# succinctlabs/kzg-rs

Measured on AMD Instinct MI355X. Metric: blobs/sec verify_blob_kzg_proof_batch, higher is better.
Workload: dtype u32 limbs (255-bit Fr / 381-bit Fp modular integers); 1 GPU; verify_blob_kzg_proof_batch, batches of 1024 synthetic blobs (4096 Fr each), device-resident, known-tau test setup (BASELINE.json configs[1]); one step = one launch group of 256 independent batches = 262144 blobs per GPU; blobs_per_gpu_per_batch=1024, batch=1024, parallelism=shard-by-blob x1, groups_in_flight=4

## Files before the change

kzg_rs_amd/csrc/capi_verify.hpp:

```cpp

static KzgRet launch_evaluate(const KzgSettings* s, const void* d_blobs, const Fr* d_z, Fr* d_y, uint32_t* d_status, size_t T, bool alone = false,
                              bool stamp = false) {
    unsigned long long* const kt = stamp && s->ws.d_ktime.p ? s->ws.d_ktime.p + 4 : nullptr;
    HIPCHK(s->d_eval_scratch.grow(eval_scratch_words(std::max<size_t>(T, 1024))));
    const unsigned per_lane = (unsigned)((T + 63) / 64);
    hipLaunchKernelGGL(k_eval_powers, dim3(per_lane), dim3(64), 0, s->s1, d_z, s->d_eval_scratch.p, (int)T);
    const unsigned eval_blocks = (unsigned)((T + EVAL_BLOBS_PER_BLOCK - 1) / EVAL_BLOBS_PER_BLOCK);
    static const long pad_opt = ab_int("eval_lds_pad", -1);
    const size_t lds_pad = pad_opt >= 0 ? (size_t)std::min(120L * 1024, pad_opt) : alone ? 0 : 16384;
    size_t spread_lds = eval_blocks <= (unsigned)s->n_cus ? (size_t)EVAL_SPREAD_LDS : lds_pad;
    if (spread_lds && DYN_LDS(k_blob_evaluate_t<true>, spread_lds) != hipSuccess) {
        (void)hipGetLastError();
        spread_lds = 0;
    }
    hipLaunchKernelGGL(k_blob_evaluate_t<true>, dim3(eval_blocks), dim3(64 * EVAL_BLOBS_PER_BLOCK), spread_lds, s->s1,
                       (const uint8_t*)d_blobs, EvalTables{s->t->d_eval_a.p, s->t->d_eval_b.p, s->t->d_eval_c.p}, s->d_eval_scratch.p, d_status, (int)T, kt);
    hipLaunchKernelGGL(k_eval_finish, dim3(per_lane), dim3(64), 0, s->s1, s->d_eval_scratch.p, s->t->d_M29.p, d_y, (int)T);
    return KZG_OK;
}

static KzgRet launch_challenge(const KzgSettings* s, const void* d_blobs, const void* d_commitments, Fr* d_z, size_t T, hipStream_t st = nullptr) {
    if (!st) st = s->s1;
    static const int forced = opt_is("challenge_kernel", "lane") ? 1 : opt_is("challenge_kernel", "split") ? 2 : opt_is("challenge_kernel", "split2") ? 3 : 0;
    const uint8_t *bl = (const uint8_t*)d_blobs, *cm = (const uint8_t*)d_commitments;
    const int form = forced ? forced : T <= 16384 ? 3 : T <= 49152 ? 2 : 1;
    s->ws.ktime_valid = false;
    if (form == 1) {
        unsigned long long* kt = s->ws.d_ktime.p;
        if (kt) {
            HIPCHK(hipMemsetAsync(kt, 0, 32, st));
            s->ws.ktime_valid = true;
        }
        hipLaunchKernelGGL(k_blob_challenge_t<4>, dim3((unsigned)((T + 255) / 256)), dim3(256), 0, st, bl, cm, d_z, (int)T, kt);
    } else if (form == 2) {
        hipLaunchKernelGGL(k_blob_challenge_split, dim3((unsigned)((T + 63) / 64)), dim3(128), 0, st, bl, cm, d_z, (int)T);
    } else {
        hipLaunchKernelGGL(k_blob_challenge_split2_t<false>, dim3((unsigned)((T + 63) / 64)), dim3(192), 0, st, bl, cm, d_z, (int)T, 0, 1024, (uint32_t*)nullptr);
    }
    HIPCHK(hipGetLastError());
    return KZG_OK;
}

enum { STAGE_NONE = 0, STAGE_BLOBS = 1, STAGE_CP = 2 };
static KzgRet ws_reserve(const KzgSettings* s, size_t T, size_t B, int stage) {
    Workspace& w = s->ws;
    if (T > w.cap_n || B > w.cap_b) {
        size_t capT = T > w.cap_n ? T : w.cap_n, capB = B > w.cap_b ? B : w.cap_b;
        w.reset();
        if (capT < 16) capT = 16;
        const size_t np = 2 * capT + 1;
        const size_t nsc = 2 * capT + capB;
        const size_t nterm = 4 * capT + 2 * capB;
        HIPCHK(w.d_z.alloc(capT));
        HIPCHK(w.d_y.alloc(capT));
        HIPCHK(w.d_scalars.alloc(nsc));
        HIPCHK(w.d_partial.alloc((capT + 255) / 256 + capB));
        HIPCHK(w.d_r.alloc(capB));
        HIPCHK(w.d_status.alloc(capT));
        HIPCHK(w.d_pflag.alloc(np));
        HIPCHK(w.d_term_point.alloc(nterm));
        HIPCHK(w.d_term_scalar.alloc(nterm));
        HIPCHK(w.d_sorted.alloc(MSM_WINDOWS * nterm));
        HIPCHK(w.d_points.alloc(np));
        HIPCHK(w.d_window.alloc(2 * MSM_WINDOWS * capB));
        HIPCHK(w.d_window_sl.alloc(2 * MSM_WINDOWS * MSM_MAX_SLICES * 4));
        HIPCHK(w.d_mult.alloc(MULT_ENTRY_BYTES * std::max((size_t)MSM_CHUNKS * np, (size_t)MSM_CHUNKS_LATENCY * std::min(np, (size_t)(2 * LATENCY_MAX_BLOBS + 1)))));
        HIPCHK(w.d_ab.alloc(2 * capB));
        HIPCHK(w.d_ktime.alloc(16));
        if (msm_affine_enabled()) HIPCHK(w.d_jtmp.alloc(np));
        HIPCHK(w.d_parts.alloc(2 * capB * MAX_WORLD));
        HIPCHK(w.d_send.alloc(2 * MAX_WORLD));
        HIPCHK(w.d_slp_in.alloc(6 * capB));
        HIPCHK(w.d_slp_out.alloc(6 * capB));
        HIPCHK(w.d_bytes.alloc(96 * np));
        HIPCHK(w.d_records.alloc(160 * capT));
        HIPCHK(w.d_sha_mid.alloc(8 * std::min(capT, (size_t)SLICED_MAX_BLOBS)));
        w.off_r = 256 * capT + 4096;
        w.off_part = w.off_r + 32 * capB;
        w.off_out = w.off_part + 288 * capB;
        w.off_parts = w.off_out + 288 * capB;
        HIPCHK(w.h_buf.alloc(w.off_parts + 288 * capB * MAX_WORLD));
        w.cap_n = capT;
        w.cap_b = capB;
    }
    const size_t n_stage = std::max<size_t>(T, 4);
    if (stage != STAGE_NONE) HIPCHK(w.d_stage_cp.grow(96 * n_stage));
    if (stage == STAGE_BLOBS) HIPCHK(w.d_stage_blobs.grow((size_t)BLOB_BYTES * n_stage));
    return KZG_OK;
}

static int msm_chunks_per_block(size_t B) {
    static const int forced = [] {
        const int v = (int)ab_int("msm_cpb", 0);
        return (v == 1 || v == 2 || v == 4) ? v : 0;
    }();
    if (forced) return forced;
    return B >= 32 ? 4 : B >= 16 ? 2 : 1;
}

static KzgRet msm_save_grow(const KzgSettings* s, size_t bytes) {
    HIPCHK(s->ws.d_msm_save.grow((bytes + 3) / 4));
    return KZG_OK;
}
static size_t msm_save_bytes(const Workspace& w) { return w.d_msm_save.cap * 4; }
static KzgRet msm_save_reserve(const KzgSettings* s, unsigned gx, unsigned gy, unsigned gz) {
    const size_t layer = msm_save_layer_bytes(gx, gy, MSM_SAVE2_WORDS);
    return msm_save_grow(s, std::max(layer, std::min(layer * gz, (size_t)512 << 20)));
}

static KzgRet run_msm(const KzgSettings* s, size_t n, size_t B) {
    Workspace& w = s->ws;
    const int T = (int)(n * B), mt = (int)(2 * n + 1);
    hipLaunchKernelGGL(k_batch_terms, dim3((unsigned)((n + 255) / 256), (unsigned)B), dim3(256), 0, s->s1, w.d_term_point.p,
                       w.d_term_scalar.p, (int)n, T, mt);
    MsmDesc d{};
    d.mult = w.d_mult.p;
    d.pflag = w.d_pflag.p;
    d.scalars = w.d_scalars.p;
    d.term_point = w.d_term_point.p;
    d.term_scalar = w.d_term_scalar.p;
    d.sorted = w.d_sorted.p;
    d.window_sums = w.d_window.p;
    d.nterms[0] = (int)n;
    d.nterms[1] = (int)(2 * n + 1);
    d.max_terms = mt;
    d.stride = 2 * T + 1;
    d.ktime = w.kstamps_valid ? w.d_ktime.p + 8 : nullptr;
    d.chunks = w.chunks;
    d.chunks_per_block = w.chunks == MSM_CHUNKS ? msm_chunks_per_block(B) : 1;
    static const int msm_flags = ab_flag("msm_xcd", true) ? MSM_FLAG_XCD : 0;
    d.flags = msm_flags;
    const unsigned slots = d.chunks / d.chunks_per_block, W = MSM_WINDOWS / d.chunks;
    unsigned S = 1;
    while (S < MSM_MAX_SLICES && W * slots * 2 * B * S < 768 && n / (2 * S) >= 1024 && 2 * S * B <= 128) S *= 2;
    static const unsigned latency_slices = [] {
        const unsigned v = (unsigned)ab_int("msm_latency_slices", 0);
        return v == 1 || v == 2 || v == 4 || v == 8 ? v : 4u;
    }();
    if (d.chunks != MSM_CHUNKS && S == 1 && n >= 256 && B <= 4) S = latency_slices;
    const size_t lds_cap = msm_lds_sort_capacity<Curve29>();
    auto slice_terms = [&](unsigned S_) { return ((size_t)mt + S_ - 1) / S_ * (size_t)d.chunks_per_block; };
    while (S < MSM_MAX_SLICES && slice_terms(S) > lds_cap && n / (2 * S) >= 1024 && 2 * S * B <= 128) S *= 2;
    const bool lds_sort = slice_terms(S) + 1 <= lds_cap;
    d.slices = (int)S;
    d.window_sums = S > 1 ? w.d_window_sl.p : w.d_window.p;
    HIPCHK(hipEventRecord(s->ev[2], s->s1));
    const int nsc = (int)(B * (2 * n + 1));
    hipLaunchKernelGGL(k_glv_split, dim3((unsigned)((nsc + 255) / 256)), dim3(256), 0, s->s1, w.d_scalars.p, nsc);
    const unsigned gz = (unsigned)(2 * B * S);
    KzgRet rc_save = msm_save_reserve(s, W, slots, gz);
    if (rc_save != KZG_OK) return rc_save;
    if (w.mult_affine) {
        if (lds_sort) msm_window_launch<Curve29Aff, true>(d, W, slots, gz, w.d_msm_save.p, msm_save_bytes(w), s->s1);
        else msm_window_launch<Curve29Aff, false>(d, W, slots, gz, w.d_msm_save.p, msm_save_bytes(w), s->s1);
    } else {
        static const bool tree_quads = ab_flag("msm_tree_quads", true);
        if (tree_quads && d.chunks != MSM_CHUNKS && B <= 4) {
            if (lds_sort) msm_window_launch<Curve29Quads, true>(d, W, slots, gz, w.d_msm_save.p, msm_save_bytes(w), s->s1);
            else msm_window_launch<Curve29Quads, false>(d, W, slots, gz, w.d_msm_save.p, msm_save_bytes(w), s->s1);
        } else if (lds_sort) msm_window_launch<Curve29, true>(d, W, slots, gz, w.d_msm_save.p, msm_save_bytes(w), s->s1);
        else msm_window_launch<Curve29, false>(d, W, slots, gz, w.d_msm_save.p, msm_save_bytes(w), s->s1);
    }
    static const bool sum_quads = ab_flag("msm_sum_quads", true);
    if (sum_quads && W == 1 && slots * S >= 2 && slots * S <= (unsigned)SUMQ_MAX_POINTS && 2 * B < 64) {
        HIPCHK(DYN_LDS(k_msm_sum_quads, SUMQ_LDS_BYTES));
        hipLaunchKernelGGL(k_msm_sum_quads, dim3((unsigned)(2 * B)), dim3(256), SUMQ_LDS_BYTES, s->s1, d.window_sums, w.d_ab.p, (int)(slots * S));
        HIPCHK(hipGetLastError());
        HIPCHK(hipEventRecord(s->ev[3], s->s1));
        return KZG_OK;
    }
    if (S > 1)
        hipLaunchKernelGGL(k_msm_fold_slices, dim3((unsigned)(2 * B * slots * W)), dim3(64), 0, s->s1, w.d_window_sl.p, w.d_window.p, (int)S, (int)W);
    if (2 * B >= 64)
        hipLaunchKernelGGL(k_msm_combine_lanes, dim3((unsigned)((2 * B + 63) / 64)), dim3(64), 0, s->s1, w.d_window.p, w.d_ab.p, (int)slots, (int)W, (int)(2 * B));
    else
        hipLaunchKernelGGL(k_msm_combine, dim3((unsigned)(2 * B)), dim3(64), 0, s->s1, w.d_window.p, w.d_ab.p, (int)slots, (int)W);
    HIPCHK(hipGetLastError());
    HIPCHK(hipEventRecord(s->ev[3], s->s1));
    return KZG_OK;
}

static KzgRet launch_decode(const KzgSettings* s, const void* d_commitments, const void* d_proofs, size_t T, bool behind_sha = true) {
    Workspace& w = s->ws;
    const int np = (int)(2 * T + 1);
    unsigned blocks = (unsigned)((2 * T + 63) / 64);
    static const bool no_latency_layout = !ab_flag("msm_latency_layout", true);
    w.chunks = (T <= LATENCY_MAX_BLOBS && !no_latency_layout) ? MSM_CHUNKS_LATENCY : MSM_CHUNKS;
    const uint8_t *c = (const uint8_t*)d_commitments, *p = (const uint8_t*)d_proofs;
    const int n2 = (int)(2 * T);
    const size_t gen_off = w.chunks == MSM_CHUNKS ? 0 : MSM_CHUNKS;
    w.mult_affine = msm_affine_enabled() && w.chunks == MSM_CHUNKS;
    if (w.mult_affine) {
        G1Aff29Mem* mult = (G1Aff29Mem*)w.d_mult.p;
        hipLaunchKernelGGL((k_g1_decode_multiples29<MSM_CHUNKS, true>), dim3((unsigned)((2 * T + 255) / 256)), dim3(256), 256 * PARK_UINT4_PER_THREAD * sizeof(uint4), s->s2, c, p, (int)T, w.d_points.p, w.d_pflag.p, w.d_mult.p, w.d_jtmp.p, n2, np,
                           w.kstamps_valid ? w.d_ktime.p + 6 : nullptr);
        const unsigned conv_blocks = (unsigned)((n2 + 64 * AFFINE_BATCH - 1) / (64 * AFFINE_BATCH));
        hipLaunchKernelGGL(k_mult_to_affine29, dim3(conv_blocks), dim3(64), 0, s->s2, w.d_jtmp.p, w.d_pflag.p, mult, n2, np);
        HIPCHK(hipEventRecord(s->ev[10], s->s2));
        hipLaunchKernelGGL(k_set_generator_multiples<G1Aff29Mem>, dim3(1), dim3(64), 0, s->s2, w.d_points.p, w.d_pflag.p, mult,
                           (const G1Aff29Mem*)s->t->d_gen_mult_aff.p, n2, np, w.chunks);
    } else {
        G1Jac29Mem* mult = (G1Jac29Mem*)w.d_mult.p;
        hipLaunchKernelGGL(k_set_generator_multiples<G1Jac29Mem>, dim3(1), dim3(64), 0, s->s2, w.d_points.p, w.d_pflag.p, mult,
                           (const G1Jac29Mem*)s->t->d_gen_mult.p + gen_off, n2, np, w.chunks);
        static const bool dec_quads = ab_flag("decode_quads", true);
        if (dec_quads && w.chunks != MSM_CHUNKS && !behind_sha && (2 * T + DECQ_POINTS_PER_BLOCK - 1) / DECQ_POINTS_PER_BLOCK <= (size_t)s->n_cus) {
            blocks = (unsigned)((2 * T + DECQ_POINTS_PER_BLOCK - 1) / DECQ_POINTS_PER_BLOCK);
            HIPCHK(DYN_LDS(k_g1_decode_multiples29_quads<MSM_CHUNKS_LATENCY>, DECQ_LDS_BYTES));
            hipLaunchKernelGGL(k_g1_decode_multiples29_quads<MSM_CHUNKS_LATENCY>, dim3(blocks), dim3(64), DECQ_LDS_BYTES, s->s2, c, p, (int)T, w.d_points.p, w.d_pflag.p, mult, n2, np);
        } else if (w.chunks == MSM_CHUNKS_LATENCY)
            hipLaunchKernelGGL((k_g1_decode_multiples29<MSM_CHUNKS_LATENCY, false>), dim3(blocks), dim3(64), 64 * PARK_UINT4_PER_THREAD * sizeof(uint4), s->s2, c, p, (int)T, w.d_points.p, w.d_pflag.p, w.d_mult.p, (G1Jac29Mem*)nullptr, n2, np);
        else
            hipLaunchKernelGGL((k_g1_decode_multiples29<MSM_CHUNKS, false>), dim3(blocks), dim3(64), 64 * PARK_UINT4_PER_THREAD * sizeof(uint4), s->s2, c, p, (int)T, w.d_points.p, w.d_pflag.p, w.d_mult.p, (G1Jac29Mem*)nullptr, n2, np);
        HIPCHK(hipEventRecord(s->ev[10], s->s2));
    }
    HIPCHK(hipGetLastError());
    return KZG_OK;
}


static void select_streams(const KzgSettings* s, size_t T) {
    if (!s->s_plain[1]) return;
    const bool small = T <= LATENCY_MAX_BLOBS;
    if (small && !s->s_half_tried) {
        s->s_half_tried = true;
        hipDeviceProp_t prop;
        if (ab_flag("cu_mask", true) && hipGetDeviceProperties(&prop, s->device) == hipSuccess && prop.multiProcessorCount >= 64) {
            const int ncu = prop.multiProcessorCount, words = (ncu + 31) / 32;
            std::vector<uint32_t> lo(words, 0), hi(words, 0);
            for (int i = 0; i < ncu; i++) ((i < ncu / 2) ? lo : hi)[i / 32] |= 1u << (i % 32);
            if (hipExtStreamCreateWithCUMask(&s->s_half[0], words, lo.data()) != hipSuccess ||
                hipExtStreamCreateWithCUMask(&s->s_half[1], words, hi.data()) != hipSuccess) {
                (void)hipGetLastError();
                if (s->s_half[0]) (void)hipStreamDestroy(s->s_half[0]);
                s->s_half[0] = s->s_half[1] = nullptr;
            }
        }
    }
    const bool use_half = small && s->s_half[0];
    s->s1 = s->s_plain[0];
    s->s_sha = use_half ? s->s_half[0] : s->s_plain[0];
    s->s2 = use_half ? s->s_half[1] : s->s_plain[1];
}
struct ScopedS2 {
    const KzgSettings* const s;
    const hipStream_t keep;
    ScopedS2(const KzgSettings* s_, hipStream_t st) : s(s_), keep(s_->s2) { s->s2 = st; }
    ScopedS2(const ScopedS2&) = delete;
    ~ScopedS2() { s->s2 = keep; }
};

struct HostBatch {
    const uint8_t *blobs, *commitments, *proofs;
    const uint8_t* z_le = nullptr;
    hostpool::Job* z_job = nullptr;
};
static size_t host_challenge_max_blobs() {
    static const size_t v = (size_t)std::max(0L, std::min(4096L, opt_int("host_challenge_max_blobs", 256)));
    return v;
}
static unsigned host_slices(size_t n) {
    static const unsigned forced = [] {
        const unsigned v = (unsigned)opt_int("host_slices", 0);
        return v == 1 || v == 2 || v == 4 || v == 8 || v == 16 ? v : 0u;
    }();
    static const bool lane_forced = opt_str("challenge_kernel") && !opt_is("challenge_kernel", "split2");
    if (n > SLICED_MAX_BLOBS || lane_forced) return 1;
    if (forced) return forced;
    return n >= 512 ? 8 : n >= 128 ? 4 : 1;
}

static KzgRet sliced_points_copy(const KzgSettings* s, const HostBatch& host, void* d_commitments, void* d_proofs, size_t T, hipEvent_t after) {
    if (!s->s_copy) {
        HIPCHK(hipStreamCreateWithFlags(&s->s_copy, hipStreamNonBlocking));
        for (auto& e : s->ev_copy) HIPCHK(hipEventCreateWithFlags(&e, hipEventDisableTiming));
    }
    if (!s->ev_slice[0])
        for (auto& e : s->ev_slice) HIPCHK(hipEventCreate(&e));
    HIPCHK(hipStreamWaitEvent(s->s_copy, after, 0));
    HIPCHK(hipMemcpyAsync(d_commitments, host.commitments, 48 * T, hipMemcpyHostToDevice, s->s_copy));
    if (d_proofs) HIPCHK(hipMemcpyAsync(d_proofs, host.proofs, 48 * T, hipMemcpyHostToDevice, s->s_copy));
    HIPCHK(hipEventRecord(s->ev_slice[0], s->s_copy));
    return KZG_OK;
}
static KzgRet sliced_segments(const KzgSettings* s, const HostBatch& host, void* d_blobs, const void* d_commitments, Fr* d_z, size_t T, unsigned S,
                              hipStream_t st) {
    s->ws.ktime_valid = false;
    HIPCHK(hipStreamWaitEvent(st, s->ev_slice[0], 0));
    const size_t W = (size_t)BLOB_BYTES / S;
    for (unsigned j = 0; j < S; j++) {
        HIPCHK(hipMemcpy2DAsync((uint8_t*)d_blobs + j * W, BLOB_BYTES, host.blobs + j * W, BLOB_BYTES, W, T, hipMemcpyHostToDevice, s->s_copy));
        HIPCHK(hipEventRecord(s->ev_slice[1 + j], s->s_copy));
        HIPCHK(hipStreamWaitEvent(st, s->ev_slice[1 + j], 0));
        hipLaunchKernelGGL(k_blob_challenge_split2_t<true>, dim3((unsigned)((T + 63) / 64)), dim3(192), 0, st, (const uint8_t*)d_blobs,
                           (const uint8_t*)d_commitments, d_z, (int)T, (int)(1024 / S * j), (int)(1024 / S * (j + 1)), s->ws.d_sha_mid.p);
    }
    HIPCHK(hipGetLastError());
    return KZG_OK;
}

static KzgRet phase1_launch_locked(const void* d_blobs, const void* d_commitments, const void* d_proofs, size_t n, size_t B,
                                   const KzgSettings* s, const HostBatch* host = nullptr) {
    if (B > MAX_BATCHES_PER_LAUNCH) return fail(KZG_BADARGS, "more than 16384 batches in one launch group");
    Workspace& w = s->ws;
    const size_t T = n * B;
    KzgRet rc;
    select_streams(s, T);
    const unsigned S = host && !host->z_le ? host_slices(T) : 1;
    w.kstamps_valid = w.d_ktime.p != nullptr;
    if (w.kstamps_valid) HIPCHK(hipMemsetAsync(w.d_ktime.p, 0, 128, s->s1));
    HIPCHK(hipEventRecord(s->ev[0], s->s1));
    if (host && S == 1) {
        HIPCHK(hipMemcpyAsync(const_cast<void*>(d_commitments), host->commitments, 48 * T, hipMemcpyHostToDevice, s->s1));
        HIPCHK(hipMemcpyAsync(const_cast<void*>(d_proofs), host->proofs, 48 * T, hipMemcpyHostToDevice, s->s1));
        HIPCHK(hipMemcpyAsync(const_cast<void*>(d_blobs), host->blobs, (size_t)BLOB_BYTES * T, hipMemcpyHostToDevice, s->s1));
        HIPCHK(hipEventRecord(s->ev[0], s->s1));
    }
    if (host && S > 1) {
        if ((rc = sliced_points_copy(s, *host, const_cast<void*>(d_commitments), const_cast<void*>(d_proofs), T, s->ev[0])) != KZG_OK) return rc;
        HIPCHK(hipStreamWaitEvent(s->s2, s->ev_slice[0], 0));
// ... 877 lines not shown
```

kzg_rs_amd/csrc/fr29_eval_fold.hpp:

```cpp
#pragma once
#include "fr29.hpp"

namespace kzg {

template <class LoadPsum>
FR29_FN Fr29 eval_sum_psums(LoadPsum psum) {
    uint64_t acc[9];
#pragma unroll
    for (int i = 0; i < 9; i++) acc[i] = 0;
    for (int k = 0; k < 64; k++) {
        const Fr29 p = psum(k);
#pragma unroll
        for (int i = 0; i < 9; i++) fr29_acc_add(acc[i], p.l[i]);
    }
    Fr29 s;
    uint64_t c = 0;
#pragma unroll
    for (int i = 0; i < 9; i++) {
        c += acc[i];
        s.l[i] = (uint32_t)c & FR29_MASK;
        c >>= 29;
    }
    const uint32_t hi = (uint32_t)c;
    c = 0;
#pragma unroll
    for (int i = 0; i < 9; i++) {
        c += s.l[i] + (uint64_t)hi * c29::FR29_ONE[i];
        s.l[i] = i < 8 ? (uint32_t)c & FR29_MASK : (uint32_t)c;
        c >>= 29;
    }
    return s;
}

template <class LoadNode, class LoadZ, class LoadRoot, class Stack>
FR29_FN Fr29 eval_fold_nodes(LoadNode node, LoadZ zpow, LoadRoot root, Stack& st) {
    Fr29 n;
    for (int k = 0; k < 64; k++) {
        n = node(k);
        int l = 0;
        for (; (k >> l) & 1; l++) {
            const Fr29 na = st.get(l);
            n = fr29_mul2(fr29_add(na, n), zpow(6 + l), fr29_sub_biased4(na, n), root((k >> l) & ~1));
        }
        if (k != 63) st.put(l, n);
    }
    return n;
}

FR29_FN Fr29 eval_tail(const Fr29& n0, const Fr29& s, const Fr29& zr, const Fr29& z4096) {
    const Fr29 sm = fr29_mul(s, fr29_const(c29::FR29_R2));
    const Fr29 x = fr29_mul(sm, z4096);
    const Fr29 nw = fr29_sub_biased(fr29_add(fr29_mul(n0, zr), sm), x);
    return fr29_mul(nw, fr29_const(c29::FR29_INV4096_PLAIN));
}

}
```

kzg_rs_amd/csrc/fr_kernels.hpp:

```cpp
#pragma once
#include "field.hpp"
#include "fr29.hpp"
#include "fr29_eval_fold.hpp"
#include "sha256.hpp"

namespace kzg {

constexpr int FE_PER_BLOB = 4096;
constexpr int BLOB_BYTES = 131072;

__device__ __forceinline__ uint32_t bitrev12(uint32_t i) { return __brev(i) >> 20; }

__global__ void k_roots_tables(Fr* __restrict__ M, Fr* __restrict__ DM) {
    int j = blockIdx.x * blockDim.x + threadIdx.x;
    if (j >= FE_PER_BLOB) return;
    uint32_t e = bitrev12(j);
    Fr w, acc = FrF::one();
#pragma unroll
    for (int i = 0; i < 8; i++) w.l[i] = consts::FR_OMEGA_MONT[i];
    for (int b = 11; b >= 0; b--) {
        acc = FrF::sqr(acc);
        if ((e >> b) & 1) acc = FrF::mul(acc, w);
    }
    M[j] = acc;
// ... 73 lines not shown
        bswap4(w, c0); bswap4(w + 4, c1); bswap4(w + 8, L[0]); bswap4(w + 12, L[1]);
        sha256_compress(st, w);
        bswap4(w, L[2]);
        w[4] = 0x80000000u;
#pragma unroll
        for (int k = 5; k < 15; k++) w[k] = 0;
        w[15] = 131152u * 8u;
        sha256_compress(st, w);
    }
    Fr d;
#pragma unroll
    for (int k = 0; k < 8; k++) d.l[k] = st.h[7 - k];
    z_out[i] = FrF::from_mont(FrF::to_mont(d));
    if (stamp) {
        const unsigned long long clk1 = __builtin_amdgcn_s_memtime(), ref1 = __builtin_amdgcn_s_memrealtime();
        atomicMax(&ktime[1], ref1);
        atomicAdd(&ktime[2], clk1 - clk0);
        atomicAdd(&ktime[3], ref1 - ref0);
    }
}

constexpr int CHALLENGE_TILE_U4 = 2 * 16 * 64;
__global__ __launch_bounds__(128) void k_blob_challenge_split(const uint8_t* __restrict__ blobs, const uint8_t* __restrict__ commitments,
                                                              Fr* __restrict__ z_out, int n) {
    __shared__ uint4 tile[CHALLENGE_TILE_U4];
    const int lane = threadIdx.x & 63;
    const int role = __builtin_amdgcn_readfirstlane(threadIdx.x >> 6);
    int i = blockIdx.x * 64 + lane;
    const bool live = i < n;
    if (!live) i = n - 1;
    constexpr int NBLK = 2050;

    if (role == 1) {
        const uint4* blob = reinterpret_cast<const uint4*>(blobs + (size_t)i * BLOB_BYTES);
        const uint4* cm = reinterpret_cast<const uint4*>(commitments + (size_t)i * 48);
        auto emit = [=](uint32_t (&w)[16], int b) {
            uint32_t kw[64];
            sha256_schedule_kw(kw, w);
            uint4* dst = tile + (b & 1) * (16 * 64) + lane;
#pragma unroll
            for (int t = 0; t < 16; t++) dst[t * 64] = make_uint4(kw[4 * t], kw[4 * t + 1], kw[4 * t + 2], kw[4 * t + 3]);
            __syncthreads();
        };
        uint4 L[8], c0, c1;
#pragma unroll
        for (int j = 0; j < 8; j++) L[j] = blob[j];
#pragma unroll 1
        for (int m = 0; m < 1024; m++) {
            uint32_t w[16];
            if (m == 0) {
                w[0] = 0x4653424c; w[1] = 0x4f425645; w[2] = 0x52494659; w[3] = 0x5f56315f;
                w[4] = 0; w[5] = 0; w[6] = 0; w[7] = FE_PER_BLOB;
            } else {
                bswap4(w, c0);
                bswap4(w + 4, c1);
            }
            bswap4(w + 8, L[0]);
            bswap4(w + 12, L[1]);
            emit(w, 2 * m);
            bswap4(w, L[2]); bswap4(w + 4, L[3]); bswap4(w + 8, L[4]); bswap4(w + 12, L[5]);
            c0 = L[6];
            c1 = L[7];
            if (m + 1 < 1024) {
                const uint4* p = blob + 8 * (m + 1);
#pragma unroll
                for (int j = 0; j < 8; j++) L[j] = p[j];
            } else {
                L[0] = cm[0]; L[1] = cm[1]; L[2] = cm[2];
            }
            emit(w, 2 * m + 1);
        }
        {
            uint32_t w[16];
            bswap4(w, c0); bswap4(w + 4, c1); bswap4(w + 8, L[0]); bswap4(w + 12, L[1]);
            emit(w, 2048);
            bswap4(w, L[2]);
            w[4] = 0x80000000u;
#pragma unroll
            for (int k = 5; k < 15; k++) w[k] = 0;
            w[15] = 131152u * 8u;
            emit(w, 2049);
        }
        __syncthreads();
    } else {
        Sha256State st;
        sha256_init(st);
        __syncthreads();
#pragma unroll 1
        for (int b = 0; b < NBLK; b++) {
            uint32_t a = st.h[0], bb = st.h[1], c = st.h[2], d = st.h[3], e = st.h[4], f = st.h[5], g = st.h[6], h = st.h[7];
            const uint4* src = tile + (b & 1) * (16 * 64) + lane;
            uint4 kw[16];
#pragma unroll
            for (int t = 0; t < 16; t++) kw[t] = src[t * 64];
#pragma unroll
            for (int t = 0; t < 16; t++) {
                asm volatile("" : "+v"(kw[t].x), "+v"(kw[t].y), "+v"(kw[t].z), "+v"(kw[t].w));
                sha256_rounds4(a, bb, c, d, e, f, g, h, kw[t]);
            }
            st.h[0] += a; st.h[1] += bb; st.h[2] += c; st.h[3] += d; st.h[4] += e; st.h[5] += f; st.h[6] += g; st.h[7] += h;
            __syncthreads();
        }
        if (live) {
            Fr dgst;
#pragma unroll
            for (int k = 0; k < 8; k++) dgst.l[k] = st.h[7 - k];
            z_out[i] = FrF::from_mont(FrF::to_mont(dgst));
        }
    }
}

template <bool SEG>
__global__ __launch_bounds__(192) void k_blob_challenge_split2_t(const uint8_t* __restrict__ blobs, const uint8_t* __restrict__ commitments,
                                                                 Fr* __restrict__ z_out, int n, int m0_arg, int m1_arg, uint32_t* __restrict__ mid) {
    __shared__ uint4 tile[CHALLENGE_TILE_U4];
    const int lane = threadIdx.x & 63;
    const int wave = __builtin_amdgcn_readfirstlane(threadIdx.x >> 6);
    const int M0 = SEG ? m0_arg : 0, M1 = SEG ? m1_arg : 1024;
    const bool last_seg = !SEG || M1 == 1024;
    const int NBLK = 2 * (M1 - M0) + (last_seg ? 2 : 0);
    if (wave == 2) {
        int i = blockIdx.x * 64 + lane;
        if (i >= n) i = n - 1;
        const uint4* blob = reinterpret_cast<const uint4*>(blobs + (size_t)i * BLOB_BYTES);
        const uint4* cm = reinterpret_cast<const uint4*>(commitments + (size_t)i * 48);
        auto emit = [=](uint32_t (&w)[16], int b) {
            uint32_t kw[64];
            sha256_schedule_kw(kw, w);
            uint4* dst = tile + (b & 1) * (16 * 64) + lane;
#pragma unroll
            for (int t = 0; t < 16; t++) dst[t * 64] = make_uint4(kw[4 * t], kw[4 * t + 1], kw[4 * t + 2], kw[4 * t + 3]);
            __syncthreads();
        };
        uint4 L[8], c0, c1;
#pragma unroll
        for (int j = 0; j < 8; j++) L[j] = blob[8 * M0 + j];
        if (SEG && M0 > 0) {
            c0 = blob[8 * M0 - 2];
            c1 = blob[8 * M0 - 1];
        }
#pragma unroll 1
        for (int m = M0; m < M1; m++) {
            uint32_t w[16];
            if (m == 0) {
                w[0] = 0x4653424c; w[1] = 0x4f425645; w[2] = 0x52494659; w[3] = 0x5f56315f;
                w[4] = 0; w[5] = 0; w[6] = 0; w[7] = FE_PER_BLOB;
            } else {
                bswap4(w, c0);
                bswap4(w + 4, c1);
            }
            bswap4(w + 8, L[0]);
            bswap4(w + 12, L[1]);
            emit(w, 2 * (m - M0));
            bswap4(w, L[2]); bswap4(w + 4, L[3]); bswap4(w + 8, L[4]); bswap4(w + 12, L[5]);
            c0 = L[6];
            c1 = L[7];
            if (m + 1 < M1) {
                const uint4* p = blob + 8 * (m + 1);
#pragma unroll
                for (int j = 0; j < 8; j++) L[j] = p[j];
            } else if (last_seg) {
                L[0] = cm[0]; L[1] = cm[1]; L[2] = cm[2];
            }
            emit(w, 2 * (m - M0) + 1);
        }
        if (last_seg) {
            uint32_t w[16];
            bswap4(w, c0); bswap4(w + 4, c1); bswap4(w + 8, L[0]); bswap4(w + 12, L[1]);
            emit(w, 2 * (M1 - M0));
            bswap4(w, L[2]);
            w[4] = 0x80000000u;
#pragma unroll
            for (int k = 5; k < 15; k++) w[k] = 0;
            w[15] = 131152u * 8u;
            emit(w, 2 * (M1 - M0) + 1);
        }
        __syncthreads();
    } else {
        const int blob_in_block = 32 * wave + 4 * (lane >> 3) + (lane & 3);
        int i = blockIdx.x * 64 + blob_in_block;
        const bool live = i < n;
        const bool a_lane = (lane & 4) == 0;
        Sha2LaneConsts c;
        c.n1 = a_lane ? 2u : 6u;
        c.n2 = a_lane ? 13u : 11u;
        c.n3 = a_lane ? 22u : 25u;
        c.m = a_lane ? 0xffffffffu : 0u;
        uint32_t H0 = a_lane ? 0x6a09e667u : 0x510e527fu, H1 = a_lane ? 0xbb67ae85u : 0x9b05688cu, H2 = a_lane ? 0x3c6ef372u : 0x1f83d9abu,
                 H3 = a_lane ? 0xa54ff53au : 0x5be0cd19u;
        uint32_t* my_mid = SEG ? mid + 8 * (size_t)(live ? i : n - 1) + (a_lane ? 0 : 4) : nullptr;
        if (SEG && M0 > 0) {
            const uint4 q = *reinterpret_cast<const uint4*>(my_mid);
            H0 = q.x; H1 = q.y; H2 = q.z; H3 = q.w;
        }
        __syncthreads();
#pragma unroll 1
        for (int b = 0; b < NBLK; b++) {
            const uint4* src = tile + (b & 1) * (16 * 64) + blob_in_block;
            constexpr int stride = 64;
            uint32_t kw[65];
#pragma unroll
            for (int t = 0; t < 16; t++) {
                const uint4 q = src[t * stride];
                kw[4 * t] = q.x; kw[4 * t + 1] = q.y; kw[4 * t + 2] = q.z; kw[4 * t + 3] = q.w;
            }
            kw[64] = 0;
            Sha2LaneRing r;
            r.x0 = H0; r.x1 = H1; r.x2 = H2; r.dd = H3;
            r.hk = a_lane ? 0u : H3 + kw[0];
            asm volatile("" : "=v"(r.nx));
#pragma unroll
            for (int t = 0; t < 6; t++) sha256_rounds10_2lane(r, kw + 10 * t + 1, c);
            sha256_rounds4_2lane(r, kw + 61, c);
            H0 += r.x0;
            H1 += r.x1;
            H2 += r.x2;
            H3 += a_lane ? r.dd : r.hk;
            __syncthreads();
        }
        if (SEG && !last_seg) {
            if (live) *reinterpret_cast<uint4*>(my_mid) = make_uint4(H0, H1, H2, H3);
            return;
        }
        const uint32_t e0 = (uint32_t)__builtin_amdgcn_update_dpp(0, (int)H0, 0x104, 0xF, 0xF, true), e1 = (uint32_t)__builtin_amdgcn_update_dpp(0, (int)H1, 0x104, 0xF, 0xF, true);
        const uint32_t e2 = (uint32_t)__builtin_amdgcn_update_dpp(0, (int)H2, 0x104, 0xF, 0xF, true), e3 = (uint32_t)__builtin_amdgcn_update_dpp(0, (int)H3, 0x104, 0xF, 0xF, true);
        if (live && a_lane) {
            const uint32_t hh[8] = {H0, H1, H2, H3, e0, e1, e2, e3};
            Fr dgst;
#pragma unroll
            for (int k = 0; k < 8; k++) dgst.l[k] = hh[7 - k];
            z_out[i] = FrF::from_mont(FrF::to_mont(dgst));
        }
    }
}

__device__ __forceinline__ Fr fr_shfl_xor(const Fr& a, int mask) {
    Fr r;
#pragma unroll
    for (int i = 0; i < 8; i++) r.l[i] = __shfl_xor((int)a.l[i], mask, 64);
    return r;
}

struct alignas(16) Fr29Mem {
    uint32_t l[12];
};
__device__ __forceinline__ Fr29 fr29_load(const Fr29Mem* p) {
    const uint4 a = *reinterpret_cast<const uint4*>(p->l), b = *reinterpret_cast<const uint4*>(p->l + 4);
    Fr29 r;
    r.l[0] = a.x; r.l[1] = a.y; r.l[2] = a.z; r.l[3] = a.w;
    r.l[4] = b.x; r.l[5] = b.y; r.l[6] = b.z; r.l[7] = b.w;
    r.l[8] = p->l[8];
    return r;
}
__global__ void k_roots_tables29(const Fr* __restrict__ M, Fr29Mem* __restrict__ M29, Fr29Mem* __restrict__ DM29) {
    int j = blockIdx.x * blockDim.x + threadIdx.x;
    if (j >= FE_PER_BLOB) return;
    Fr w = FrF::from_mont(M[j]);
    const Fr29 r2 = fr29_const(c29::FR29_R2);
    Fr29 m = fr29_mul(fr29_from_words(w.l), r2), dm = fr29_mul(m, r2);
#pragma unroll
    for (int i = 0; i < 12; i++) {
        M29[j].l[i] = i < 9 ? m.l[i] : 0u;
        DM29[j].l[i] = i < 9 ? dm.l[i] : 0u;
    }
}

constexpr int EVAL_SLOTS = 63;
struct EvalTables {
    const uint4 *a, *b;
    const uint32_t* c;
};
__global__ void k_eval_tables(const Fr29Mem* __restrict__ M29, const Fr29Mem* __restrict__ DM29, uint4* __restrict__ ta,
                              uint4* __restrict__ tb, uint32_t* __restrict__ tc) {
    const int slot = blockIdx.x, lane = threadIdx.x;
    const Fr29Mem* e;
    if (slot < 32) {
        e = DM29 + 2 * (32 * lane + slot);
    } else {
        int L = 1, rel = slot - 32;
        while (rel >= (32 >> L)) { rel -= 32 >> L; L++; }
        const int q = (rel << L) | ((1 << L) - 1);
        e = M29 + (((32 * lane + q) >> (L - 1)) & ~1);
    }
    ta[slot * 64 + lane] = make_uint4(e->l[0], e->l[1], e->l[2], e->l[3]);
    tb[slot * 64 + lane] = make_uint4(e->l[4], e->l[5], e->l[6], e->l[7]);
    tc[slot * 64 + lane] = e->l[8];
}

struct EvalRsrc {
    __amdgpu_buffer_rsrc_t a, b, c;
};
__device__ __forceinline__ Fr29 eval_table_load(const EvalRsrc& t, int slot, uint32_t lane16, uint32_t lane4) {
    typedef uint32_t u32x4 __attribute__((ext_vector_type(4)));
    const u32x4 a = __builtin_amdgcn_raw_buffer_load_b128(t.a, lane16, slot * 1024, 0);
    const u32x4 b = __builtin_amdgcn_raw_buffer_load_b128(t.b, lane16, slot * 1024, 0);
    Fr29 r;
    r.l[0] = a.x; r.l[1] = a.y; r.l[2] = a.z; r.l[3] = a.w;
    r.l[4] = b.x; r.l[5] = b.y; r.l[6] = b.z; r.l[7] = b.w;
    r.l[8] = __builtin_amdgcn_raw_buffer_load_b32(t.c, lane4, slot * 256, 0);
    return r;
}

constexpr int EVAL_SCRATCH_WORDS = 14 * 9;
constexpr int EVAL_NODE_WORDS = 2 * 64 * 12;
__host__ __device__ inline size_t eval_nodes_offset(size_t T) { return (T * EVAL_SCRATCH_WORDS + 3) & ~(size_t)3; }
__host__ __device__ inline size_t eval_scratch_words(size_t T) { return eval_nodes_offset(T) + T * EVAL_NODE_WORDS; }
__global__ __launch_bounds__(64) void k_eval_powers(const Fr* __restrict__ z_in, uint32_t* __restrict__ scratch, int T) {
    const int b = blockIdx.x * 64 + threadIdx.x;
    if (b >= T) return;
    const Fr zin = z_in[b];
    const Fr29 r2 = fr29_const(c29::FR29_R2);
    Fr29* Z = reinterpret_cast<Fr29*>(scratch + (size_t)b * EVAL_SCRATCH_WORDS);
    Fr29 z = fr29_mul(fr29_from_words(zin.l), r2);
    Z[0] = z;
    Z[13] = fr29_mul(z, r2);
    for (int l = 1; l <= 12; l++) {
        z = fr29_mul(z, z);
        Z[l] = z;
    }
}
__global__ __launch_bounds__(64) void k_eval_finish(const uint32_t* __restrict__ scratch, const Fr29Mem* __restrict__ M29, Fr* __restrict__ y_out, int T) {
    __shared__ uint32_t zs[6][9][64], stack[6][9][64];
    const int lane = threadIdx.x, b = blockIdx.x * 64 + lane;
    if (b >= T) return;
    const uint32_t* Z = scratch + (size_t)b * EVAL_SCRATCH_WORDS;
    const Fr29Mem* nodes = reinterpret_cast<const Fr29Mem*>(scratch + eval_nodes_offset(T)) + (size_t)b * 128;
    for (int L = 6; L < 12; L++)
#pragma unroll
        for (int i = 0; i < 9; i++) zs[L - 6][i][lane] = Z[L * 9 + i];
    struct Stack {
        uint32_t (*s)[9][64];
        int lane;
        __device__ Fr29 get(int l) const {
            Fr29 r;
#pragma unroll
            for (int i = 0; i < 9; i++) r.l[i] = s[l][i][lane];
            return r;
        }
        __device__ void put(int l, const Fr29& n) {
#pragma unroll
            for (int i = 0; i < 9; i++) s[l][i][lane] = n.l[i];
        }
    } st{stack, lane};
    const Fr29 sum = eval_sum_psums([&](int k) { return fr29_load(nodes + 64 + k); });
    const Fr29 n0 = eval_fold_nodes([&](int k) { return fr29_load(nodes + k); },
                                    [&](int L) {
                                        Fr29 r;
#pragma unroll
                                        for (int i = 0; i < 9; i++) r.l[i] = zs[L - 6][i][lane];
                                        return r;
                                    },
                                    [&](int j) {
                                        Fr29 r;
#pragma unroll
                                        for (int i = 0; i < 9; i++) r.l[i] = M29[j].l[i];
                                        return r;
                                    },
                                    st);
    const Fr29* Zp = reinterpret_cast<const Fr29*>(Z);
    const Fr29 y29 = eval_tail(n0, sum, Zp[0], Zp[12]);
    Fr y;
    fr29_to_words(y.l, y29);
    y_out[b] = FrF::reduce_once(y);
}

constexpr int EVAL_BLOBS_PER_BLOCK = 4;
constexpr int EVAL_SPREAD_LDS = 96 * 1024;
template <bool SPLIT>
__global__ __launch_bounds__(256, 3) void k_blob_evaluate_t(const uint8_t* __restrict__ blobs, const EvalTables tab,
                                                       uint32_t* __restrict__ scratch, uint32_t* __restrict__ status, int T,
                                                       unsigned long long* __restrict__ ktime) {
    static_assert(SPLIT, "k_blob_evaluate_t has one form");
    const int wave = threadIdx.x >> 6, lane = threadIdx.x & 63;
    const int blob_idx = blockIdx.x * EVAL_BLOBS_PER_BLOCK + wave;
    const bool active = blob_idx < T;
    __shared__ Fr29 Zs[EVAL_BLOBS_PER_BLOCK][14];
    __shared__ uint4 stack_as[EVAL_BLOBS_PER_BLOCK][4][64], stack_bs[EVAL_BLOBS_PER_BLOCK][4][64];
    __shared__ uint32_t stack_cs[EVAL_BLOBS_PER_BLOCK][4][64];
    Fr29* Z = Zs[wave];
    uint4 (*stack_a)[64] = stack_as[wave], (*stack_b)[64] = stack_bs[wave];
    uint32_t (*stack_c)[64] = stack_cs[wave];
    if (!active) return;
    kstamp_in(ktime);
    const int blob_u = __builtin_amdgcn_readfirstlane(blob_idx);
    uint32_t* const my = scratch + (size_t)blob_u * EVAL_SCRATCH_WORDS;
    for (int i = lane; i < 14 * 9; i += 64) reinterpret_cast<uint32_t*>(Z)[i] = my[i];
    const Fr29 zd = Z[13];
    bool bad = false;
    Fr29 n, psum;
#pragma unroll
    for (int i = 0; i < 9; i++) psum.l[i] = 0;
    uint4 cur[8];
    const __amdgpu_buffer_rsrc_t rs_blob = __builtin_amdgcn_make_buffer_rsrc(const_cast<uint8_t*>(blobs) + (size_t)blob_u * BLOB_BYTES, 0, BLOB_BYTES, 0x00020000);
    EvalRsrc rs;
    rs.a = __builtin_amdgcn_make_buffer_rsrc(const_cast<uint4*>(tab.a), 0, EVAL_SLOTS * 64 * 16, 0x00020000);
    rs.b = __builtin_amdgcn_make_buffer_rsrc(const_cast<uint4*>(tab.b), 0, EVAL_SLOTS * 64 * 16, 0x00020000);
    rs.c = __builtin_amdgcn_make_buffer_rsrc(const_cast<uint32_t*>(tab.c), 0, EVAL_SLOTS * 64 * 4, 0x00020000);
    const uint32_t lane2k = (uint32_t)lane * 2048u, lane16 = (uint32_t)lane * 16u, lane4 = (uint32_t)lane * 4u;
    auto blob_load = [&](int byte_off) {
        typedef uint32_t u32x4 __attribute__((ext_vector_type(4)));
        const u32x4 v = __builtin_amdgcn_raw_buffer_load_b128(rs_blob, lane2k, byte_off, 0);
        return make_uint4(v.x, v.y, v.z, v.w);
    };
#pragma unroll
    for (int i = 0; i < 8; i++) cur[i] = blob_load(16 * i);
    Fr29 leaf0 = eval_table_load(rs, 0, lane16, lane4), leaf1 = eval_table_load(rs, 1, lane16, lane4);
    struct PairOps {
        Fr29 s, u;
    };
    auto convert = [&](const uint4& a_hi, const uint4& a_lo, const uint4& b_hi, const uint4& b_lo) {
        Fr wa = fr_from_be_words(a_hi, a_lo), wb = fr_from_be_words(b_hi, b_lo);
        if (__any((wa.l[7] >= consts::FR_MOD[7]) | (wb.l[7] >= consts::FR_MOD[7]))) bad |= FrF::geq_mod(wa) | FrF::geq_mod(wb);
        const Fr29 pa = fr29_from_words(wa.l), pb = fr29_from_words(wb.l);
        PairOps o;
        o.s = fr29_add(pa, pb);
        o.u = fr29_sub_biased4(pa, pb);
        psum = fr29_add(psum, o.s);
        return o;
    };
    for (int j = 0; j < 16; j++) {
        const int jn = j < 15 ? j + 1 : 15;
        const PairOps p0 = convert(cur[0], cur[1], cur[2], cur[3]);
        __builtin_amdgcn_sched_barrier(0x7);
#pragma unroll
        for (int i = 0; i < 4; i++) cur[i] = blob_load(128 * jn + 16 * i);
        __builtin_amdgcn_sched_barrier(0x7);
        const Fr29 n0 = fr29_mul2(p0.s, zd, p0.u, leaf0);
        const PairOps p1 = convert(cur[4], cur[5], cur[6], cur[7]);
        __builtin_amdgcn_sched_barrier(0x7);
#pragma unroll
        for (int i = 4; i < 8; i++) cur[i] = blob_load(128 * jn + 16 * i);
        Fr29 root = eval_table_load(rs, 32 + j, lane16, lane4);
        __builtin_amdgcn_sched_barrier(0x7);
        const Fr29 n1 = fr29_mul2(p1.s, zd, p1.u, leaf1);
        psum = fr29_normalize(psum);
        __builtin_amdgcn_sched_barrier(0x7);
        leaf0 = eval_table_load(rs, 2 * jn, lane16, lane4);
        leaf1 = eval_table_load(rs, 2 * jn + 1, lane16, lane4);
        Fr29 root_next = eval_table_load(rs, 48 + (j >> 1), lane16, lane4);
        __builtin_amdgcn_sched_barrier(0x7);
        n = fr29_mul2(fr29_add(n0, n1), Z[1], fr29_sub_biased4(n0, n1), root);
        root = root_next;
        int level = 2;
        for (int jj = j; jj & 1; jj >>= 1) {
            Fr29 na;
            const uint4 h0 = stack_a[level - 2][lane], h1 = stack_b[level - 2][lane];
            na.l[0] = h0.x; na.l[1] = h0.y; na.l[2] = h0.z; na.l[3] = h0.w;
            na.l[4] = h1.x; na.l[5] = h1.y; na.l[6] = h1.z; na.l[7] = h1.w;
            na.l[8] = stack_c[level - 2][lane];
            root_next = eval_table_load(rs, 64 - (32 >> level) + (j >> level), lane16, lane4);
            const Fr29 sum = fr29_add(na, n), dif = fr29_sub_biased4(na, n);
            n = fr29_mul2(sum, Z[level], dif, root);
            root = root_next;
            level++;
        }
        if (j != 15) {
            stack_a[level - 2][lane] = make_uint4(n.l[0], n.l[1], n.l[2], n.l[3]);
            stack_b[level - 2][lane] = make_uint4(n.l[4], n.l[5], n.l[6], n.l[7]);
            stack_c[level - 2][lane] = n.l[8];
        }
    }
    {
        uint32_t* const mine = scratch + eval_nodes_offset((size_t)T) + (size_t)blob_u * EVAL_NODE_WORDS;
        const __amdgpu_buffer_rsrc_t rs_n = __builtin_amdgcn_make_buffer_rsrc(mine, 0, EVAL_NODE_WORDS * 4, 0x00020000);
        typedef uint32_t u32x4 __attribute__((ext_vector_type(4)));
        const uint32_t entry = (uint32_t)lane * 48u;
        auto put = [&](const Fr29& v, int kind_off) {
            __builtin_amdgcn_raw_buffer_store_b128(u32x4{v.l[0], v.l[1], v.l[2], v.l[3]}, rs_n, entry, kind_off, 0);
            __builtin_amdgcn_raw_buffer_store_b128(u32x4{v.l[4], v.l[5], v.l[6], v.l[7]}, rs_n, entry + 16, kind_off, 0);
            __builtin_amdgcn_raw_buffer_store_b32(v.l[8], rs_n, entry + 32, kind_off, 0);
        };
        put(n, 0);
        put(psum, 64 * 48);
    }
    const unsigned long long any_bad = __ballot(bad);
    if (lane == 0 && any_bad) atomicOr(&status[blob_u], 1u);
    kstamp_out(ktime);
}

__device__ __forceinline__ Fr fr_shfl(const Fr& a, int src) {
    Fr r;
#pragma unroll
    for (int i = 0; i < 8; i++) r.l[i] = __shfl((int)a.l[i], src, 64);
    return r;
}
__device__ inline Fr fr_inverse_mont(const Fr& a) {
    return pow_limbs<Fr, 8>(a, consts::FR_R_MINUS_2, FrF::one(), [](const Fr& x, const Fr& y) { return FrF::mul(x, y); });
}
__global__ __launch_bounds__(64) void k_blob_quotient(const uint8_t* __restrict__ blobs, const Fr* __restrict__ z_in,
                                                      const Fr* __restrict__ y_in, const Fr* __restrict__ M, Fr* __restrict__ out,
                                                      uint32_t* __restrict__ status) {
    const int b = blockIdx.x, lane = threadIdx.x;
    const Fr zM = FrF::to_mont(z_in[b]), y = y_in[b];
    const uint4* src = reinterpret_cast<const uint4*>(blobs + (size_t)b * BLOB_BYTES) + (size_t)lane * 128;
    Fr* o = out + (size_t)b * FE_PER_BLOB + 64 * lane;
    const Fr* Ml = M + 64 * lane;
    Fr acc = FrF::one();
    int special = -1;
    for (int k = 0; k < 64; k++) {
        Fr d = FrF::sub(Ml[k], zM);
        if (FrF::is_zero(d)) {
            special = k;
            d = FrF::one();
        }
        o[k] = acc;
        acc = FrF::mul(acc, d);
    }
    Fr incl = acc;
    for (int sh = 1; sh < 64; sh <<= 1) {
        Fr up = fr_shfl(incl, lane >= sh ? lane - sh : lane);
        if (lane >= sh) incl = FrF::mul(incl, up);
    }
    const Fr total = fr_shfl(incl, 63);
    Fr excl = fr_shfl(incl, lane ? lane - 1 : 0);
    if (lane == 0) excl = FrF::one();
    const Fr inv_total = fr_inverse_mont(total);
    Fr sfx = acc;
    for (int sh = 1; sh < 64; sh <<= 1) {
        Fr dn = fr_shfl(sfx, lane + sh < 64 ? lane + sh : lane);
        if (lane + sh < 64) sfx = FrF::mul(sfx, dn);
    }
    Fr sfx_excl = fr_shfl(sfx, lane < 63 ? lane + 1 : 63);
    if (lane == 63) sfx_excl = FrF::one();
    Fr running = FrF::mul(inv_total, sfx_excl);
    bool bad = false;
    Fr wsum = FrF::zero();
    for (int k = 63; k >= 0; k--) {
        Fr d = FrF::sub(Ml[k], zM);
        if (k == special) d = FrF::one();
        const Fr inv_d = FrF::mul(running, FrF::mul(excl, o[k]));
        running = FrF::mul(running, d);
        const Fr p = fr_from_be_words(src[2 * k], src[2 * k + 1]);
        bad |= FrF::geq_mod(p);
        Fr q = FrF::mul(FrF::sub(p, y), inv_d);
        if (k == special) q = FrF::zero();
        o[k] = q;
        wsum = FrF::add(wsum, FrF::mul(q, Ml[k]));
    }
    const unsigned long long any_special = __ballot(special >= 0);
    if (any_special) {
        for (int sh = 1; sh < 64; sh <<= 1) wsum = FrF::add(wsum, fr_shfl_xor(wsum, sh));
        if (special >= 0) o[special] = FrF::neg(FrF::mul(wsum, fr_inverse_mont(zM)));
    }
    if (__ballot(bad) && lane == 0) atomicOr(&status[b], 1u);
}

}
```

Measured before the change: 4.877 million blobs/s.

## Parallelize eval finish across 8 lanes per blob with DPP folds, pre-reduce psums

```diff
diff --git a/kzg_rs_amd/csrc/capi_verify.hpp b/kzg_rs_amd/csrc/capi_verify.hpp
--- a/kzg_rs_amd/csrc/capi_verify.hpp
+++ b/kzg_rs_amd/csrc/capi_verify.hpp
@@ -15,7 +15,8 @@
     }
     hipLaunchKernelGGL(k_blob_evaluate_t<true>, dim3(eval_blocks), dim3(64 * EVAL_BLOBS_PER_BLOCK), spread_lds, s->s1,
                        (const uint8_t*)d_blobs, EvalTables{s->t->d_eval_a.p, s->t->d_eval_b.p, s->t->d_eval_c.p}, s->d_eval_scratch.p, d_status, (int)T, kt);
-    hipLaunchKernelGGL(k_eval_finish, dim3(per_lane), dim3(64), 0, s->s1, s->d_eval_scratch.p, s->t->d_M29.p, d_y, (int)T);
+    const unsigned finish_blocks = (unsigned)((T + EVAL_FINISH_BLOBS_PER_BLOCK - 1) / EVAL_FINISH_BLOBS_PER_BLOCK);
+    hipLaunchKernelGGL(k_eval_finish, dim3(finish_blocks), dim3(8 * EVAL_FINISH_BLOBS_PER_BLOCK), 0, s->s1, s->d_eval_scratch.p, s->t->d_M29.p, d_y, (int)T);
     return KZG_OK;
 }
 
diff --git a/kzg_rs_amd/csrc/fr29_eval_fold.hpp b/kzg_rs_amd/csrc/fr29_eval_fold.hpp
--- a/kzg_rs_amd/csrc/fr29_eval_fold.hpp
+++ b/kzg_rs_amd/csrc/fr29_eval_fold.hpp
@@ -47,6 +47,61 @@
     return n;
 }
 
+FR29_FN Fr29 eval_merge(const Fr29& na, const Fr29& nb, const Fr29& zl, const Fr29& w) {
+    return fr29_mul2(fr29_add(na, nb), zl, fr29_sub_biased4(na, nb), w);
+}
+
+FR29_FN int eval_root8_index(int L, int j, int i) { return ((8 * j) >> (L - 6)) + 2 * i; }
+template <class LoadNode, class LoadRoot>
+FR29_FN Fr29 eval_fold8(LoadNode node, const Fr29& z6, const Fr29& z7, const Fr29& z8, LoadRoot root) {
+    const Fr29 a0 = eval_merge(node(0), node(1), z6, root(6, 0));
+    const Fr29 a1 = eval_merge(node(2), node(3), z6, root(6, 1));
+    const Fr29 b0 = eval_merge(a0, a1, z7, root(7, 0));
+    const Fr29 a2 = eval_merge(node(4), node(5), z6, root(6, 2));
+    const Fr29 a3 = eval_merge(node(6), node(7), z6, root(6, 3));
+    const Fr29 b1 = eval_merge(a2, a3, z7, root(7, 1));
+    return eval_merge(b0, b1, z8, root(8, 0));
+}
+FR29_FN int eval_root_cross_index(int t, int j) { return 2 * (j >> (t + 1)); }
+
+struct EvalPsum {
+    uint32_t l[10];
+};
+FR29_FN EvalPsum eval_psum_split(const Fr29& p) {
+    EvalPsum r;
+#pragma unroll
+    for (int i = 0; i < 8; i++) r.l[i] = p.l[i];
+    r.l[8] = p.l[8] & FR29_MASK;
+    r.l[9] = p.l[8] >> 29;
+    return r;
+}
+FR29_FN EvalPsum eval_psum_add(const EvalPsum& a, const EvalPsum& b) {
+    EvalPsum r;
+#pragma unroll
+    for (int i = 0; i < 10; i++) r.l[i] = a.l[i] + b.l[i];
+    return r;
+}
+FR29_FN EvalPsum eval_psum_normalize(const EvalPsum& a) {
+    EvalPsum r = a;
+#pragma unroll
+    for (int i = 0; i < 9; i++) {
+        r.l[i + 1] += r.l[i] >> 29;
+        r.l[i] &= FR29_MASK;
+    }
+    return r;
+}
+FR29_FN Fr29 eval_psum_fold(const EvalPsum& a) {
+    Fr29 s;
+    uint64_t c = 0;
+#pragma unroll
+    for (int i = 0; i < 9; i++) {
+        c += a.l[i] + (uint64_t)a.l[9] * c29::FR29_ONE[i];
+        s.l[i] = i < 8 ? (uint32_t)c & FR29_MASK : (uint32_t)c;
+        c >>= 29;
+    }
+    return s;
+}
+
 FR29_FN Fr29 eval_tail(const Fr29& n0, const Fr29& s, const Fr29& zr, const Fr29& z4096) {
     const Fr29 sm = fr29_mul(s, fr29_const(c29::FR29_R2));
     const Fr29 x = fr29_mul(sm, z4096);
diff --git a/kzg_rs_amd/csrc/fr_kernels.hpp b/kzg_rs_amd/csrc/fr_kernels.hpp
--- a/kzg_rs_amd/csrc/fr_kernels.hpp
+++ b/kzg_rs_amd/csrc/fr_kernels.hpp
@@ -399,7 +399,7 @@
 }
 
 constexpr int EVAL_SCRATCH_WORDS = 14 * 9;
-constexpr int EVAL_NODE_WORDS = 2 * 64 * 12;
+constexpr int EVAL_NODE_WORDS = (64 + 8) * 12;
 __host__ __device__ inline size_t eval_nodes_offset(size_t T) { return (T * EVAL_SCRATCH_WORDS + 3) & ~(size_t)3; }
 __host__ __device__ inline size_t eval_scratch_words(size_t T) { return eval_nodes_offset(T) + T * EVAL_NODE_WORDS; }
 __global__ __launch_bounds__(64) void k_eval_powers(const Fr* __restrict__ z_in, uint32_t* __restrict__ scratch, int T) {
@@ -416,49 +416,81 @@
         Z[l] = z;
     }
 }
-__global__ __launch_bounds__(64) void k_eval_finish(const uint32_t* __restrict__ scratch, const Fr29Mem* __restrict__ M29, Fr* __restrict__ y_out, int T) {
-    __shared__ uint32_t zs[6][9][64], stack[6][9][64];
-    const int lane = threadIdx.x, b = blockIdx.x * 64 + lane;
-    if (b >= T) return;
-    const uint32_t* Z = scratch + (size_t)b * EVAL_SCRATCH_WORDS;
-    const Fr29Mem* nodes = reinterpret_cast<const Fr29Mem*>(scratch + eval_nodes_offset(T)) + (size_t)b * 128;
-    for (int L = 6; L < 12; L++)
-#pragma unroll
-        for (int i = 0; i < 9; i++) zs[L - 6][i][lane] = Z[L * 9 + i];
-    struct Stack {
-        uint32_t (*s)[9][64];
-        int lane;
-        __device__ Fr29 get(int l) const {
-            Fr29 r;
-#pragma unroll
-            for (int i = 0; i < 9; i++) r.l[i] = s[l][i][lane];
-            return r;
-        }
-        __device__ void put(int l, const Fr29& n) {
-#pragma unroll
-            for (int i = 0; i < 9; i++) s[l][i][lane] = n.l[i];
-        }
-    } st{stack, lane};
-    const Fr29 sum = eval_sum_psums([&](int k) { return fr29_load(nodes + 64 + k); });
-    const Fr29 n0 = eval_fold_nodes([&](int k) { return fr29_load(nodes + k); },
-                                    [&](int L) {
-                                        Fr29 r;
-#pragma unroll
-                                        for (int i = 0; i < 9; i++) r.l[i] = zs[L - 6][i][lane];
-                                        return r;
-                                    },
-                                    [&](int j) {
-                                        Fr29 r;
-#pragma unroll
-                                        for (int i = 0; i < 9; i++) r.l[i] = M29[j].l[i];
-                                        return r;
-                                    },
-                                    st);
-    const Fr29* Zp = reinterpret_cast<const Fr29*>(Z);
-    const Fr29 y29 = eval_tail(n0, sum, Zp[0], Zp[12]);
-    Fr y;
-    fr29_to_words(y.l, y29);
-    y_out[b] = FrF::reduce_once(y);
+constexpr int DPP_XOR1 = 0xB1, DPP_XOR2 = 0x4E, DPP_SHL4 = 0x104;
+template <int CTRL, int N>
+__device__ __forceinline__ void dpp_words(uint32_t (&o)[N], const uint32_t (&a)[N]) {
+#pragma unroll
+    for (int i = 0; i < N; i++) o[i] = (uint32_t)__builtin_amdgcn_update_dpp(0, (int)a[i], CTRL, 0xF, 0xF, true);
+}
+__device__ __forceinline__ EvalPsum eval_psum_gather8(EvalPsum p) {
+    EvalPsum o;
+    dpp_words<DPP_XOR1>(o.l, p.l);
+    p = eval_psum_add(p, o);
+    dpp_words<DPP_XOR2>(o.l, p.l);
+    p = eval_psum_add(p, o);
+    dpp_words<DPP_SHL4>(o.l, p.l);
+    return eval_psum_add(p, o);
+}
+__device__ __forceinline__ Fr29 fr29_load_packed(const uint32_t* p) {
+    typedef uint32_t u32x4p __attribute__((ext_vector_type(4), aligned(4)));
+    const u32x4p a = *reinterpret_cast<const u32x4p*>(p), b = *reinterpret_cast<const u32x4p*>(p + 4);
+    Fr29 r;
+    r.l[0] = a.x; r.l[1] = a.y; r.l[2] = a.z; r.l[3] = a.w;
+    r.l[4] = b.x; r.l[5] = b.y; r.l[6] = b.z; r.l[7] = b.w;
+    r.l[8] = p[8];
+    return r;
+}
+constexpr int EVAL_FINISH_BLOBS_PER_BLOCK = 32;
+__global__ __launch_bounds__(256) void k_eval_finish(const uint32_t* __restrict__ scratch, const Fr29Mem* __restrict__ M29, Fr* __restrict__ y_out, int T) {
+    const int j = threadIdx.x & 7, b = blockIdx.x * EVAL_FINISH_BLOBS_PER_BLOCK + (threadIdx.x >> 3);
+    if (blockIdx.x * EVAL_FINISH_BLOBS_PER_BLOCK + ((threadIdx.x >> 6) << 3) >= T) return;
+    const bool live = b < T;
+    const size_t bs = live ? (size_t)b : 0;
+    const uint32_t* Z = scratch + bs * EVAL_SCRATCH_WORDS;
+    const Fr29Mem* nodes = reinterpret_cast<const Fr29Mem*>(scratch + eval_nodes_offset(T)) + bs * (EVAL_NODE_WORDS / 12);
+    auto zero = [] {
+        Fr29 r;
+#pragma unroll
+        for (int i = 0; i < 9; i++) r.l[i] = 0;
+        return r;
+    };
+    auto zpow = [&](int L) {
+        Fr29 r = zero();
+        if (live) r = fr29_load_packed(Z + 9 * L);
+        return r;
+    };
+    EvalPsum ps;
+#pragma unroll
+    for (int i = 0; i < 10; i++) ps.l[i] = 0;
+    if (live) {
+        const Fr29Mem* e = nodes + 64 + j;
+        const Fr29 lo = fr29_load(e);
+#pragma unroll
+        for (int i = 0; i < 9; i++) ps.l[i] = lo.l[i];
+        ps.l[9] = e->l[9];
+    }
+    ps = eval_psum_normalize(eval_psum_gather8(eval_psum_normalize(ps)));
+    const Fr29 sum = eval_psum_fold(ps);
+    Fr29 n = eval_fold8([&](int i) {
+                            Fr29 r = zero();
+                            if (live) r = fr29_load(nodes + 8 * j + i);
+                            return r;
+                        },
+                        zpow(6), zpow(7), zpow(8),
+                        [&](int L, int i) { return fr29_load(M29 + eval_root8_index(L, j, i)); });
+    Fr29 o;
+    dpp_words<DPP_XOR1>(o.l, n.l);
+    n = eval_merge(n, o, zpow(9), fr29_load(M29 + eval_root_cross_index(0, j)));
+    dpp_words<DPP_XOR2>(o.l, n.l);
+    n = eval_merge(n, o, zpow(10), fr29_load(M29 + eval_root_cross_index(1, j)));
+    dpp_words<DPP_SHL4>(o.l, n.l);
+    n = eval_merge(n, o, zpow(11), fr29_load(M29 + eval_root_cross_index(2, j)));
+    const Fr29 y29 = eval_tail(n, sum, zpow(0), zpow(12));
+    if (live && j == 0) {
+        Fr y;
+        fr29_to_words(y.l, y29);
+        y_out[b] = FrF::reduce_once(y);
+    }
 }
 
 constexpr int EVAL_BLOBS_PER_BLOCK = 4;
@@ -561,14 +593,18 @@
         uint32_t* const mine = scratch + eval_nodes_offset((size_t)T) + (size_t)blob_u * EVAL_NODE_WORDS;
         const __amdgpu_buffer_rsrc_t rs_n = __builtin_amdgcn_make_buffer_rsrc(mine, 0, EVAL_NODE_WORDS * 4, 0x00020000);
         typedef uint32_t u32x4 __attribute__((ext_vector_type(4)));
+        typedef uint32_t u32x2 __attribute__((ext_vector_type(2)));
         const uint32_t entry = (uint32_t)lane * 48u;
-        auto put = [&](const Fr29& v, int kind_off) {
-            __builtin_amdgcn_raw_buffer_store_b128(u32x4{v.l[0], v.l[1], v.l[2], v.l[3]}, rs_n, entry, kind_off, 0);
-            __builtin_amdgcn_raw_buffer_store_b128(u32x4{v.l[4], v.l[5], v.l[6], v.l[7]}, rs_n, entry + 16, kind_off, 0);
-            __builtin_amdgcn_raw_buffer_store_b32(v.l[8], rs_n, entry + 32, kind_off, 0);
-        };
-        put(n, 0);
-        put(psum, 64 * 48);
+        __builtin_amdgcn_raw_buffer_store_b128(u32x4{n.l[0], n.l[1], n.l[2], n.l[3]}, rs_n, entry, 0, 0);
+        __builtin_amdgcn_raw_buffer_store_b128(u32x4{n.l[4], n.l[5], n.l[6], n.l[7]}, rs_n, entry + 16, 0, 0);
+        __builtin_amdgcn_raw_buffer_store_b32(n.l[8], rs_n, entry + 32, 0, 0);
+        const EvalPsum p8 = eval_psum_gather8(eval_psum_split(psum));
+        if ((lane & 7) == 0) {
+            const uint32_t pe = (uint32_t)(lane >> 3) * 48u;
+            __builtin_amdgcn_raw_buffer_store_b128(u32x4{p8.l[0], p8.l[1], p8.l[2], p8.l[3]}, rs_n, pe, 64 * 48, 0);
+            __builtin_amdgcn_raw_buffer_store_b128(u32x4{p8.l[4], p8.l[5], p8.l[6], p8.l[7]}, rs_n, pe + 16, 64 * 48, 0);
+            __builtin_amdgcn_raw_buffer_store_b64(u32x2{p8.l[8], p8.l[9]}, rs_n, pe + 32, 64 * 48, 0);
+        }
     }
     const unsigned long long any_bad = __ballot(bad);
     if (lane == 0 && any_bad) atomicOr(&status[blob_u], 1u);
```

Result: slower. 4.589 million blobs/s (-5.9%).
